# raider99k/UNINA-YOLO-DLA

Hardware: AMD Instinct MI355X
Metric: frames/sec, 640x640 batch-1 (p99 latency alongside) (higher is better)
Workload: dtype f16; 1 GPU; unina-yolo-dla-m graph A fp16, batch=1, 640x640, NMS on-GPU (BASELINE configs[1]); frames_in_flight_per_gpu=2, parallelism=1 GPU, distinct_frames=2048, detections_last_frame=446

## Files before the change

### unina-yolo-dla_amd/csrc/conv_igemm.hip

```cpp
#include "kernels.h"
#include "block_pipeline.h"

#include <cstdlib>

namespace unina {

using namespace dev;

namespace {

typedef float floatx4_t __attribute__((ext_vector_type(4)));

__device__ __forceinline__ void tile_of_block(const ConvParams& p, int orig, int nwg, int* bx, int* by) {
  const int q = nwg >> 3, r = nwg & 7, xcd = orig & 7;
  const int v = (xcd < r ? xcd * (q + 1) : r * (q + 1) + (xcd - r) * q) + (orig >> 3);
  const bool mm = p.xcd_m_major != 0;
  const int major = fast_div(v, mm ? p.gn_magic : p.gm_magic);
  const int minor = v - major * (mm ? p.grid_n : p.grid_m);
  *bx = mm ? major : minor;
  *by = mm ? minor : major;
}

__device__ __forceinline__ void stamp_entry(const ConvParams& p, long long t) {
  if (p.stamps && blockIdx.x == (gridDim.x >> 1) && threadIdx.x == 0) p.stamps[7] = t;
}

__device__ __forceinline__ void stamp_now(const ConvParams& p, int k) {
  p.stamps[k] = __builtin_amdgcn_s_memtime();
  if (k == 0 || k == 4) p.stamps[5 + (k >> 2)] = wall_clock64();
}
__device__ __forceinline__ void stamp(const ConvParams& p, int k) {
  if (p.stamps && blockIdx.x == (gridDim.x >> 1) && threadIdx.x == 0) stamp_now(p, k);
}
__device__ __forceinline__ void stamp(const ConvParams& p, int k, int bid, int nwg) {
  if (p.stamps && bid == (nwg >> 1) && threadIdx.x == 0) stamp_now(p, k);
}

__device__ __forceinline__ void stamp_wg(const ConvParams& p, int which) {
  if (p.wg_times && threadIdx.x == 0) p.wg_times[2 * blockIdx.x + which] = wall_clock64();
}

typedef int intx4 __attribute__((ext_vector_type(4)));
template <typename T> struct Elem;
template <> struct Elem<half_t> {
  static constexpr int kChunk = 8, kBlockK = 32, kPlanes = 1;
  static constexpr int kDType = kF16;
  static constexpr const char* kTag = "f16";
  typedef half8 frag;
  typedef floatx4 acc_t;
  static __device__ __forceinline__ acc_t mma(const frag& a, const frag& b, acc_t c) {
    return __builtin_amdgcn_mfma_f32_16x16x32_f16(a, b, c, 0, 0, 0);
  }
  static __device__ __forceinline__ floatx4 to_float(const acc_t& c) { return c; }
  static __device__ __forceinline__ frag lds(const unsigned char* at, int) { return *reinterpret_cast<const frag*>(at); }
};
template <> struct Elem<s16_t> {
  static constexpr int kChunk = 8, kBlockK = 32, kPlanes = 2;
  static constexpr int kDType = kS16;
  static constexpr const char* kTag = "s16";
  typedef half8x2 frag;
  typedef floatx4 acc_t;
  static __device__ __forceinline__ acc_t mma(const frag& a, const frag& b, acc_t c) { return mfma_split(a, b, c); }
  static __device__ __forceinline__ floatx4 to_float(const acc_t& c) { return c; }
  static __device__ __forceinline__ frag lds(const unsigned char* at, int lo_off) {
    return frag{*reinterpret_cast<const half8*>(at), *reinterpret_cast<const half8*>(at + lo_off)};
  }
};
template <> struct Elem<float> {
  static constexpr int kChunk = 4, kBlockK = 16, kPlanes = 1;
  static constexpr int kDType = kF32;
  static constexpr const char* kTag = "f32";
  static __device__ __forceinline__ floatx4_t lds(const unsigned char* at, int) { return *reinterpret_cast<const floatx4_t*>(at); }
  typedef floatx4_t frag;
  typedef floatx4 acc_t;
  static __device__ __forceinline__ acc_t mma(const frag& a, const frag& b, acc_t c) {
#pragma unroll
    for (int e = 0; e < 4; ++e) c = __builtin_amdgcn_mfma_f32_16x16x4f32(a[e], b[e], c, 0, 0, 0);
    return c;
  }
  static __device__ __forceinline__ floatx4 to_float(const acc_t& c) { return c; }
};
template <> struct Elem<signed char> {
  static constexpr int kChunk = 16, kBlockK = 64, kPlanes = 1;
  static constexpr int kDType = kI8;
// ... 530 lines not shown
      const int h = h00[i] + tap_off;
      hrow[i] = h << (nch_log + 4);
      hsw[i] = h & swz;
    }
#pragma unroll
    for (int j = 0; j < KSUB; ++j) {
      const int ch = (cs * KSUB + j) * 4 + lq;
#pragma unroll
      for (int i = 0; i < WM_T; ++i) f.b[j][i] = *reinterpret_cast<const frag_t*>(patch + hrow[i] + ((ch ^ hsw[i]) << 4));
#pragma unroll
      for (int n = 0; n < WN_T; ++n) f.a[j][n] = *reinterpret_cast<const frag_t*>(sb + (((wn * WN_T + n) * KSUB + j) << 10));
    }
  };
  auto mma_frags = [&](const Frags& f) {
#pragma unroll
    for (int j = 0; j < KSUB; ++j)
#pragma unroll
      for (int n = 0; n < WN_T; ++n)
#pragma unroll
        for (int i = 0; i < WM_T; ++i) acc[n][i] = E::mma(f.a[j][n], f.b[j][i], acc[n][i]);
  };
  EpiConsts<WN_T> ec;
  load_epi_consts<WN_T>(sg, nb0 + wn * (WN_T * 16), lq, ec);
  Frags fa, fb;
  wait_stages<LPT>(n_pro - 1);
  __builtin_amdgcn_s_barrier();
  read_frags(fa, 0);
  stamp(p, 2);
  int kt = 0;
  for (; kt + STAGES < nk; kt += 2) {
    wait_vmcnt<(STAGES - 3) * LPT>();
    __builtin_amdgcn_s_barrier();
    issue((kt + STAGES - 1) % STAGES);
    read_frags(fb, kt + 1);
    mma_frags(fa);
    wait_vmcnt<(STAGES - 3) * LPT>();
    __builtin_amdgcn_s_barrier();
    issue((kt + STAGES) % STAGES);
    read_frags(fa, kt + 2);
    mma_frags(fb);
  }
  bool cur_a = true;
  for (; kt < nk; ++kt) {
    if (kt + 1 < nk) {
      const int issued = kt + STAGES - 1 < nk ? kt + STAGES - 1 : nk;
      wait_stages<LPT>(issued - (kt + 2));
      __builtin_amdgcn_s_barrier();
      if (kt + STAGES - 1 < nk) issue((kt + STAGES - 1) % STAGES);
      if (cur_a) {
        read_frags(fb, kt + 1);
        mma_frags(fa);
      } else {
        read_frags(fa, kt + 1);
        mma_frags(fb);
      }
    } else if (cur_a) {
      mma_frags(fa);
    } else {
      mma_frags(fb);
    }
    cur_a = !cur_a;
  }
  wait_vmcnt<0>();
  stamp(p, 3);

  conv_epilogue<T, BM, BN, WM_T, WN_T>(p, sg, acc, ec, wm, wn, nb0, l15, lq,
                                       [&](int pl) {
                                         const int oy = ty0 + pl / TW, ox = tx0 + pl % TW;
                                         return (oy < p.Ho && ox < p.Wo) ? oy * p.Wo + ox : -1;
                                       },
                                       conv_smem);
  if (p.stamps) {
    asm volatile("s_waitcnt vmcnt(0)" ::: "memory");
    stamp(p, 4);
  }
}
template <typename T, int TH, int TW, int BN, int BK, int WAVES_M, int WAVES_N, int STAGES>
constexpr auto kernel_of(HaloTile<T, TH, TW, BN, BK, WAVES_M, WAVES_N, STAGES>) { return conv3x3_halo<T, TH, TW, BN, BK, WAVES_M, WAVES_N, STAGES>; }

#ifndef UNINA_PATCH_VIA_REGS
#define UNINA_PATCH_VIA_REGS 1
#endif
constexpr bool kPatchViaRegs = UNINA_PATCH_VIA_REGS != 0;
template <typename T, int TH, int TW, int BN, int CIN, int NW, int D, int S = 1>
struct RegqTile : TileDefaults {
  typedef T elem;
  static constexpr int bm = TH * TW, bn = BN, bk = 32, stages = 3, th = TH, tw = TW, cin = CIN, nthreads = NW * 64, stride = S;
  static constexpr int nw = NW, depth = D;
  static constexpr bool SPLIT = Elem<T>::kPlanes == 2;
  static constexpr int R0W = S * (TW - 1) + 3, R0H = S * (TH - 1) + 3;
  static constexpr int PATCH = (int)round_kib(R0H * R0W * CIN * sizeof(T)) + 1024;
  static constexpr int LDS_LO = SPLIT ? PATCH : 0;
  static constexpr size_t lds_bytes(int = 0) { return SPLIT ? 2 * (size_t)PATCH : max_sz(PATCH, stage_bytes((bm + 15) & ~15, BN)); }
  static constexpr Str name() {
    return Str() << "conv3x3_regq<" << Elem<T>::kTag << "," << TH << "x" << TW << "," << BN << "," << CIN << "," << NW << (S == 2 ? "w,s2>" : "w>");
  }
};

template <int TH, int TW, int BN, int CIN, int NW, int D, int S = 1, int WN = 1, typename T = half_t, bool STAMPS = false>
__device__ __forceinline__ void conv3x3_regq_body(const ConvParams& p, int bid, int nwg) {
  typedef Elem<T> E;
  typedef typename E::frag frag;
  typedef RegqTile<T, TH, TW, BN, CIN, NW, D, S> Tile;
  constexpr bool SPLIT = Tile::SPLIT;
  typedef typename std::conditional<sizeof(T) == 1, EltI8, typename std::conditional<SPLIT, EltS, EltH>::type>::type PE;
  constexpr int BM = TH * TW, R0W = Tile::R0W, R0H = Tile::R0H, NT = NW * 64, CB = CIN / E::kBlockK, KB = 9 * CB;
  static_assert(CIN % E::kBlockK == 0, "a weight block must not straddle a tap");
  constexpr int NS = BN / 16 / WN, WVM = NW / NS, MS = (BM + 15) / 16, WM_T = (MS + WVM - 1) / WVM;
  static_assert((BN / 16) % WN == 0 && NW % NS == 0 && WM_T >= 1 && KB * WN >= D, "tile");

  if constexpr (STAMPS) { stamp(p, 0, bid, nwg); stamp_wg(p, 0); }
  const int lane = threadIdx.x & 63;
  const int wid = __builtin_amdgcn_readfirstlane(threadIdx.x >> 6);
  const int wm = wid / NS, wn = wid % NS;
  const int l15 = lane & 15, lq = lane >> 4;
  int bx, by;
  tile_of_block(p, bid, nwg, &bx, &by);
  const int sidx = (p.nseg > 1 && by >= p.seg[1].tile0) ? 1 : 0;
  const ConvSeg& sg = p.seg[sidx];
  const int n_pad = (sg.n_count + 15) & ~15;
  const int nb0 = (by - sg.tile0) * BN;
  const int tiles_x = (p.Wo + TW - 1) / TW;
  const int tyi = fast_div(bx, p.tx_magic), txi = bx - tyi * tiles_x;
  const int ty0 = tyi * TH, tx0 = txi * TW;

  const unsigned char* wptr[WN];
#pragma unroll
  for (int j = 0; j < WN; ++j) {
    int nsub = (nb0 >> 4) + wn * WN + j;
    nsub = nsub * 16 < n_pad ? nsub : (n_pad >> 4) - 1;
    wptr[j] = static_cast<const unsigned char*>(sg.w_lane) + (size_t)nsub * KB * PE::WBLK + lane * 16;
  }
  frag q[D];
  auto fetch = [&](auto gc) {
    constexpr int g = decltype(gc)::value;
    if constexpr (g < KB * WN) q[g % D] = PE::ldw(wptr[g % WN] + (g / WN) * PE::WBLK);
  };
  constexpr int LDS_LO = Tile::LDS_LO;

  constexpr Img X = make_img(0, CIN / E::kChunk);
  if constexpr (SPLIT) {
    load_patch<R0H, R0W, CIN, NT, PE>(conv_smem, static_cast<const T*>(p.src) + sg.src_coff, p.src_ld, p.H, p.W, S * ty0 - 1,
                                      S * tx0 - 1, p.zeros, wid, lane, p.src_lo, LDS_LO);
    static_for<0, D>(fetch);
  } else if constexpr (kPatchViaRegs) {
    PatchRegs<R0H, R0W, CIN, NT, PE> pr;
    patch_issue<R0H, R0W, CIN, NT, PE>(pr, static_cast<const T*>(p.src) + sg.src_coff, p.src_ld, p.H, p.W, S * ty0 - 1, S * tx0 - 1, wid, lane);
    static_for<0, D>(fetch);
    if constexpr (STAMPS) stamp(p, 1, bid, nwg);
    patch_commit<R0H, R0W, CIN, NT, PE>(pr, conv_smem, wid, lane);
  } else {
    load_patch<R0H, R0W, CIN, NT, PE>(conv_smem, static_cast<const T*>(p.src) + sg.src_coff, p.src_ld, p.H, p.W, S * ty0 - 1,
                                      S * tx0 - 1, p.zeros, wid, lane);
    static_for<0, D>(fetch);
  }
  EpiConsts<WN> ec;
  load_epi_consts<WN>(sg, nb0 + wn * (WN * 16), lq, ec);
  if constexpr (STAMPS && (SPLIT || !kPatchViaRegs)) stamp(p, 1, bid, nwg);
  if constexpr (SPLIT || !kPatchViaRegs) asm volatile("s_waitcnt vmcnt(0)" ::: "memory");
  lds_barrier();
  if constexpr (STAMPS) stamp(p, 2, bid, nwg);

  int row0[WM_T];
#pragma unroll
  for (int i = 0; i < WM_T; ++i) {
    int pp = (wm * WM_T + i) * 16 + l15;
    pp = pp < BM ? pp : BM - 1;
    row0[i] = S * ((pp / TW) * R0W + pp % TW);
  }
  auto baddr = [&](int i, auto kc) {
    constexpr int kb = decltype(kc)::value, tap = kb / CB, cb = kb - tap * CB, th3 = tap / 3;
    return X.addr(row0[i] + th3 * R0W + (tap - th3 * 3), cb * 4 + lq);
  };
  typename E::acc_t acc[WN][WM_T];
  frag b[2][WM_T];
#pragma unroll
  for (int i = 0; i < WM_T; ++i) {
#pragma unroll
    for (int j = 0; j < WN; ++j) acc[j][i] = typename E::acc_t{0, 0, 0, 0};
    b[0][i] = PE::ld(conv_smem + baddr(i, std::integral_constant<int, 0>{}), LDS_LO);
  }
  static_for<0, KB>([&](auto kc) {
    constexpr int kb = decltype(kc)::value;
    frag a[WN];
#pragma unroll
    for (int j = 0; j < WN; ++j) a[j] = q[(kb * WN + j) % D];
    static_for<0, WN>([&](auto jc) { fetch(std::integral_constant<int, kb * WN + decltype(jc)::value + D>{}); });
    if constexpr (kb + 1 < KB) {
#pragma unroll
      for (int i = 0; i < WM_T; ++i) b[(kb + 1) & 1][i] = PE::ld(conv_smem + baddr(i, std::integral_constant<int, kb + 1>{}), LDS_LO);
    }
#pragma unroll
    for (int j = 0; j < WN; ++j)
#pragma unroll
      for (int i = 0; i < WM_T; ++i) acc[j][i] = E::mma(a[j], b[kb & 1][i], acc[j][i]);
  });

  if constexpr (STAMPS) stamp(p, 3, bid, nwg);
  auto pix_to_m = [&](int pl) {
    const int oy = ty0 + pl / TW, ox = tx0 + pl % TW;
    return (pl < BM && oy < p.Ho && ox < p.Wo) ? oy * p.Wo + ox : -1;
  };
  conv_epilogue<T, BM, BN, WM_T, WN, decltype(pix_to_m), (UNINA_REGQ_DIRECT_STORE != 0 && sizeof(T) == 2)>(p, sg, acc, ec, wm, wn, nb0, l15, lq, pix_to_m,
                                                                                                       conv_smem, NT);
  if constexpr (STAMPS) { stamp(p, 4, bid, nwg); asm volatile("s_waitcnt vmcnt(0)" ::: "memory"); stamp_wg(p, 1); }
}

template <int TH, int TW, int BN, int CIN, int NW, int D, int S = 1, int WN = 1, typename T = half_t>
__global__ __launch_bounds__(NW * 64) void conv3x3_regq(const ConvParams p) {
  conv3x3_regq_body<TH, TW, BN, CIN, NW, D, S, WN, T>(p, (int)blockIdx.x, (int)gridDim.x);
}
template <typename T, int TH, int TW, int BN, int CIN, int NW, int D, int S>
constexpr auto kernel_of(RegqTile<T, TH, TW, BN, CIN, NW, D, S>) { return conv3x3_regq<TH, TW, BN, CIN, NW, D, S, 1, T>; }

template <typename T, int TH, int CIN, int NCHUNK, int NW>
struct WsTile : TileDefaults {
  typedef T elem;
  static constexpr int TW = 16, BN = NW * 16;
  static constexpr int bm = TH * TW, bn = BN, bk = 32, stages = 3, th = TH, tw = TW, cin = CIN, nthreads = NW * 64, chunks = NCHUNK;
  static constexpr int nw = NW;
  static constexpr bool ws = true;
  static constexpr int ESZ = sizeof(T) == 1 ? 1 : 2;
  static constexpr int R0W = TW + 2, R0H = TH + 2, CC = CIN / NCHUNK;
  static constexpr int PITCH = CC * ESZ + 32;
  static constexpr int PLANE = R0H * R0W * PITCH;
  static constexpr int BUF = Elem<T>::kPlanes * PLANE;
  static constexpr size_t lds_bytes(int = 0) { return (size_t)(NCHUNK > 1 ? 2 : 1) * BUF; }
  static constexpr Str name() {
    return Str() << "conv3x3_ws<" << Elem<T>::kTag << "," << TH << "x16," << CIN << "/" << NCHUNK << "," << NW << "w>";
  }
};

template <typename T, int TH, int CIN, int NCHUNK, int NW, bool STAMPS = false>
__device__ __forceinline__ void conv3x3_wsc_body(const ConvParams& p, int bid, int nwg) {
  typedef Elem<T> E;
  typedef typename E::frag frag;
  typedef WsTile<T, TH, CIN, NCHUNK, NW> Tile;
  constexpr bool SP = E::kPlanes == 2;
  constexpr bool I8 = sizeof(T) == 1;
  constexpr int ESZ = Tile::ESZ, KBLK = E::kBlockK;
  constexpr int WB = 1024 * E::kPlanes;
  if constexpr (STAMPS) { stamp(p, 0, bid, nwg); stamp_wg(p, 0); }
  typedef unsigned uintx4 __attribute__((ext_vector_type(4)));
  typedef float floatx2 __attribute__((ext_vector_type(2)));
  constexpr int TW = Tile::TW, R0W = Tile::R0W, R0H = Tile::R0H, NT = NW * 64, BN = Tile::BN;
  constexpr int CB = CIN / KBLK, CC = Tile::CC, CBC = CC / KBLK, KBC = 9 * CBC;
  constexpr int STEPS = R0H * 3 * CBC, PF = 4;
  constexpr int PITCH = Tile::PITCH, PLANE = Tile::PLANE, BUF = Tile::BUF;
  static_assert(CIN % (KBLK * NCHUNK) == 0 && KBC * 4 * E::kPlanes <= 160 && PLANE % 16 == 0, "chunking: two weight sets must fit the registers");
  static_assert((R0H * R0W + 2) * PITCH < 65536, "ds_read immediate offsets");
  const int lane = threadIdx.x & 63;
  const int wid = __builtin_amdgcn_readfirstlane(threadIdx.x >> 6);
  const int l15 = lane & 15, lq = lane >> 4;
  int bx, by;
  tile_of_block(p, bid, nwg, &bx, &by);
  const int sidx = (p.nseg > 1 && by >= p.seg[1].tile0) ? 1 : 0;
  const ConvSeg& sg = p.seg[sidx];
  const int n_pad = (sg.n_count + 15) & ~15;
  const int nb0 = (by - sg.tile0) * BN;
  const int tiles_x = (p.Wo + TW - 1) / TW;
  const int tyi = fast_div(bx, p.tx_magic), txi = bx - tyi * tiles_x;
  const int ty0 = tyi * TH, tx0 = txi * TW;

  int nsub = (nb0 >> 4) + wid;
  nsub = nsub * 16 < n_pad ? nsub : (n_pad >> 4) - 1;
  const unsigned char* wptr = static_cast<const unsigned char*>(sg.w_lane) + (size_t)nsub * (9 * CB) * WB + lane * 16;
  const int n = nb0 + wid * 16 + lq * 4;
  const bool n_ok = n < sg.n_count;
  const floatx4 bias = *reinterpret_cast<const floatx4*>(sg.bias + (n_ok ? n : 0));

  const int src_bytes = p.H * p.W * p.src_ld * ESZ;
  const __amdgpu_buffer_rsrc_t srs_h = __builtin_amdgcn_make_buffer_rsrc(const_cast<void*>(p.src), 0, src_bytes, 0x00020000);
  const __amdgpu_buffer_rsrc_t srs_l =
      __builtin_amdgcn_make_buffer_rsrc(const_cast<unsigned char*>(static_cast<const unsigned char*>(p.src) + (SP ? p.src_lo : 0)), 0, src_bytes, 0x00020000);
  constexpr int nchx = CC * ESZ / 16, nslots = R0H * R0W * nchx, PITER = (nslots + NT - 1) / NT;

  const bool out16 = !I8 || sg.out_dtype == kF16;
  const int DSZ = out16 ? 2 : 1;
  const unsigned rowb = (unsigned)(p.Wo * sg.dst_ld * DSZ);
  const __amdgpu_buffer_rsrc_t drs_h = __builtin_amdgcn_make_buffer_rsrc(sg.dst, 0, (int)((unsigned)p.Ho * rowb), 0x00020000);
  const __amdgpu_buffer_rsrc_t drs_l =
      __builtin_amdgcn_make_buffer_rsrc(static_cast<unsigned char*>(sg.dst) + (SP ? sg.dst_lo : 0), 0, (int)((unsigned)p.Ho * rowb), 0x00020000);
  const bool lane_ok = n_ok && tx0 + l15 < p.Wo;
  const unsigned voff0 = lane_ok ? (unsigned)(((ty0 * p.Wo + tx0 + l15) * sg.dst_ld + n) * DSZ) : 0x40000000u;
  floatx4 mult = {1.f, 1.f, 1.f, 1.f};
  if constexpr (I8) mult = *reinterpret_cast<const floatx4*>(sg.mult + (n_ok ? n : 0));
  const float out_inv = sg.out_inv_scale;

  typename E::acc_t acc[TH];
  auto store_row = [&](auto rc) {
    constexpr int r = decltype(rc)::value;
    if constexpr (!I8) {
      const floatx4 v = acc[r] + bias;
      half4 hv, lv;
#pragma unroll
      for (int e = 0; e < 4; ++e) {
// ... 101 lines not shown
      }
      if constexpr (s + PF < STEPS) b[(s + PF) % (PF + 1)] = bfrag(std::integral_constant<int, s + PF>{});
      if constexpr (ch == 0 && kx == 0 && cbl == 0 && rho < TH) acc[rho] = typename E::acc_t{0, 0, 0, 0};
      if constexpr (SP) {
        static_for<0, 3>([&](auto tc) {
          constexpr int term = decltype(tc)::value;
          static_for<0, 3>([&](auto kyc) {
            constexpr int ky = decltype(kyc)::value, r = rho - ky;
            if constexpr (r >= 0 && r < TH) {
              const auto& wv = w[(ky * 3 + kx) * CBC + cbl];
              const auto& bv = b[s % (PF + 1)];
              acc[r] = __builtin_amdgcn_mfma_f32_16x16x32_f16(term == 0 ? wv.l : wv.h, term == 1 ? bv.l : bv.h, acc[r], 0, 0, 0);
            }
          });
        });
      } else {
        static_for<0, 3>([&](auto kyc) {
          constexpr int ky = decltype(kyc)::value, r = rho - ky;
          if constexpr (r >= 0 && r < TH) acc[r] = E::mma(w[(ky * 3 + kx) * CBC + cbl], b[s % (PF + 1)], acc[r]);
        });
      }
      if constexpr (ch == NCHUNK - 1 && kx == 1 && cbl == 0 && rho >= 3) store_row(std::integral_constant<int, rho - 3>{});
      __builtin_amdgcn_sched_barrier(0);
    });
    if constexpr (ch + 1 < NCHUNK) {
      patch_commit((ch + 1) & 1);
      lds_barrier();
    }
  });
  if constexpr (STAMPS) stamp(p, 3, bid, nwg);
  store_row(std::integral_constant<int, TH - 1>{});
  if constexpr (STAMPS) { stamp(p, 4, bid, nwg); asm volatile("s_waitcnt vmcnt(0)" ::: "memory"); stamp_wg(p, 1); }
}

template <typename T, int TH, int CIN, int NCHUNK, int NW>
__global__ __launch_bounds__(NW * 64) void conv3x3_wsc(const ConvParams p) {
  conv3x3_wsc_body<T, TH, CIN, NCHUNK, NW>(p, (int)blockIdx.x, (int)gridDim.x);
}
template <typename T, int TH, int CIN, int NCHUNK, int NW>
constexpr auto kernel_of(WsTile<T, TH, CIN, NCHUNK, NW>) { return conv3x3_wsc<T, TH, CIN, NCHUNK, NW>; }

template <typename T> using WsP3 = WsTile<T, 16, 128, (Elem<T>::kPlanes == 2 ? 4 : 2), 4>;
template <typename T> using WsP4 = WsTile<T, 8, 256, 4, 4>;
typedef WsTile<half_t, 8, 128, 2, 4> WsP3Half;
typedef WsTile<half_t, 4, 256, 4, 4> WsP4Half;

template <class A, class B, bool STAMPS = false, int MIN_WAVES = 0>
__global__ __launch_bounds__(A::nthreads, MIN_WAVES) void conv_dual_ws(const ConvParams pa, const ConvParams pb, int nb) {
  if ((int)blockIdx.x < nb) conv3x3_wsc_body<typename B::elem, B::th, B::cin, B::chunks, B::nw, STAMPS>(pb, (int)blockIdx.x, nb);
  else conv3x3_wsc_body<typename A::elem, A::th, A::cin, A::chunks, A::nw, STAMPS>(pa, (int)blockIdx.x - nb, (int)gridDim.x - nb);
}

#ifndef UNINA_CONV_PROBE
template <typename T> using RegqP3 = RegqTile<T, 8, 16, 64, 128, 8, 8>;
template <typename T> using RegqP4 = RegqTile<T, 8, 8, 64, 256, 8, 8>;

template <class A, class B>
__global__ __launch_bounds__(A::nthreads, A::SPLIT ? 0 : 4) void conv_dual_regq(const ConvParams pa, const ConvParams pb, int na) {
  if ((int)blockIdx.x < na) conv3x3_regq_body<A::th, A::tw, A::bn, A::cin, A::nw, A::depth, A::stride, 1, typename A::elem>(pa, (int)blockIdx.x, na);
  else conv3x3_regq_body<B::th, B::tw, B::bn, B::cin, B::nw, B::depth, B::stride, 1, typename B::elem>(pb, (int)blockIdx.x - na, (int)gridDim.x - na);
}

typedef GldsTile<half_t, 128, 16, 64, 4, 1, 4> Head1x1;
__global__ __launch_bounds__(256) void conv_dual_head1x1(const ConvParams pa, const ConvParams pb, int na) {
  if ((int)blockIdx.x < na) conv_glds_body<half_t, 128, 16, 64, 4, 1, 4>(pa, (int)blockIdx.x, na);
  else conv_glds_body<half_t, 128, 16, 64, 4, 1, 4>(pb, (int)blockIdx.x - na, (int)gridDim.x - na);
}

namespace {

constexpr int kCUs = 256;

struct CfgInfo {
  int bm = 0, bn = 0, bk = 0, stages = 0;
  Str name = Str() << "n/a";
  void (*fn)(const ConvParams) = nullptr;
  size_t (*lds_bytes)(int cin) = nullptr;
  int th = 0, tw = 0;
  int cin = 0;
  int nthreads = 0;
  int stride = 0;
  bool ws = false;
  int chunks = 0;
};
struct ConvTable {
  CfgInfo at[kNumDTypes][kCfgCount];
  int clashes = 0;
  template <class Tile>
  constexpr void add(ConvConfig cfg) {
    CfgInfo& c = at[Elem<typename Tile::elem>::kDType][cfg];
    if (c.fn) ++clashes;
    c = {Tile::bm, Tile::bn, Tile::bk, Tile::stages, Tile::name(), kernel_of(Tile{}), &Tile::lds_bytes,
         Tile::th, Tile::tw, Tile::cin, Tile::nthreads, Tile::stride, Tile::ws, Tile::chunks};
  }
};

template <typename T, int ST>
constexpr void add_glds(ConvTable& t) {
  t.add<GldsTile<T, 64, 64, 64, 2, 2, ST>>(kCfg64x64k64);
  t.add<GldsTile<T, 64, 64, 32, 2, 2, 4>>(kCfg64x64k32);
  t.add<GldsTile<T, 128, 64, 64, 2, 2, ST>>(kCfg128x64k64);
  t.add<GldsTile<T, 128, 64, 32, 2, 2, 4>>(kCfg128x64k32);
  t.add<GldsTile<T, 128, 32, 64, 4, 1, ST>>(kCfg128x32k64);
  t.add<GldsTile<T, 128, 32, 32, 4, 1, 4>>(kCfg128x32k32);
  t.add<GldsTile<T, 128, 16, 64, 4, 1, ST>>(kCfg128x16k64);
  t.add<GldsTile<T, 32, 64, 64, 1, 4, 4>>(kCfg32x64k64);
}
template <typename T>
constexpr void add_glds_halo(ConvTable& t) {
  add_glds<T, 4>(t);
  t.add<GldsTile<T, 128, 128, 64, 2, 2, 4>>(kCfg128x128k64);
  t.add<GldsTile<T, 32, 64, 64, 1, 4, 8>>(kCfg32x64k64s8);
  t.add<GldsTile<T, 64, 64, 64, 2, 2, 6>>(kCfg64x64k64s6);
  t.add<HaloTile<T, 8, 8, 64, 64, 2, 2, 4>>(kCfgHalo8x8n64);
  t.add<HaloTile<T, 8, 8, 32, 64, 4, 1, 4>>(kCfgHalo8x8n32);
  t.add<HaloTile<T, 8, 16, 64, 64, 2, 2, 4>>(kCfgHalo8x16n64);
  t.add<HaloTile<T, 8, 16, 32, 64, 4, 1, 4>>(kCfgHalo8x16n32);
  t.add<HaloTile<T, 8, 8, 64, 32, 2, 2, 4>>(kCfgHalo8x8n64k32);
  t.add<HaloTile<T, 8, 16, 32, 32, 4, 1, 4>>(kCfgHalo8x16n32k32);
  t.add<GldsTile<T, 32, 64, 128, 1, 4, 4>>(kCfg32x64k128);
  t.add<GldsTile<T, 64, 64, 128, 2, 2, 4>>(kCfg64x64k128);
}

constexpr ConvTable conv_table() {
  ConvTable t;
  add_glds_halo<half_t>(t);
  add_glds_halo<float>(t);
  add_glds_halo<signed char>(t);
  add_glds<s16_t, 3>(t);

  t.add<RegqTile<half_t, 8, 16, 64, 128, 8, 16>>(kCfgRegq8x16n64c128);
  t.add<RegqTile<half_t, 8, 8, 64, 128, 8, 16>>(kCfgRegq8x8n64c128);
  t.add<RegqTile<half_t, 8, 8, 64, 256, 8, 16>>(kCfgRegq8x8n64c256);
  t.add<RegqTile<half_t, 8, 8, 32, 256, 8, 16>>(kCfgRegq8x8n32c256);
  t.add<RegqTile<half_t, 8, 16, 64, 64, 8, 16>>(kCfgRegq8x16n64c64);
  t.add<RegqTile<half_t, 8, 16, 32, 128, 8, 16>>(kCfgRegq8x16n32c128);
  t.add<RegqTile<half_t, 8, 8, 64, 64, 8, 16, 2>>(kCfgRegqS2_8x8n64c64);
  t.add<RegqTile<half_t, 8, 16, 64, 64, 8, 16, 2>>(kCfgRegqS2_8x16n64c64);
  t.add<RegqTile<half_t, 8, 8, 64, 128, 8, 16, 2>>(kCfgRegqS2_8x8n64c128);
  t.add<RegqTile<half_t, 4, 8, 64, 128, 8, 16, 2>>(kCfgRegqS2_4x8n64c128);
  t.add<RegqTile<half_t, 8, 16, 64, 32, 8, 8, 2>>(kCfgRegqS2_8x16n64c32);
  t.add<RegqTile<half_t, 8, 8, 32, 128, 8, 16, 2>>(kCfgRegqS2_8x8n32c128);
  t.add<RegqTile<signed char, 8, 16, 64, 128, 8, 16>>(kCfgRegq8x16n64c128);
  t.add<RegqTile<signed char, 8, 8, 64, 128, 8, 16>>(kCfgRegq8x8n64c128);
  t.add<RegqTile<signed char, 8, 8, 64, 256, 8, 16>>(kCfgRegq8x8n64c256);
  t.add<RegqTile<signed char, 8, 8, 32, 256, 8, 16>>(kCfgRegq8x8n32c256);
  t.add<RegqTile<signed char, 8, 16, 32, 128, 8, 16>>(kCfgRegq8x16n32c128);
  t.add<RegqTile<signed char, 8, 8, 64, 64, 8, 8, 2>>(kCfgRegqS2_8x8n64c64);
  t.add<RegqTile<signed char, 8, 16, 64, 64, 8, 8, 2>>(kCfgRegqS2_8x16n64c64);
  t.add<RegqTile<signed char, 8, 8, 64, 128, 8, 16, 2>>(kCfgRegqS2_8x8n64c128);
  t.add<RegqTile<signed char, 4, 8, 64, 128, 8, 16, 2>>(kCfgRegqS2_4x8n64c128);
  t.add<RegqTile<signed char, 8, 8, 32, 128, 8, 16, 2>>(kCfgRegqS2_8x8n32c128);
  t.add<RegqTile<s16_t, 8, 16, 64, 128, 8, 8>>(kCfgRegq8x16n64c128);
  t.add<RegqTile<s16_t, 8, 8, 64, 128, 8, 8>>(kCfgRegq8x8n64c128);
  t.add<RegqTile<s16_t, 8, 8, 64, 256, 8, 8>>(kCfgRegq8x8n64c256);
  t.add<RegqTile<s16_t, 8, 16, 64, 64, 8, 8>>(kCfgRegq8x16n64c64);
  t.add<RegqTile<s16_t, 8, 8, 64, 64, 8, 8, 2>>(kCfgRegqS2_8x8n64c64);
  t.add<RegqTile<s16_t, 8, 8, 64, 128, 8, 8, 2>>(kCfgRegqS2_8x8n64c128);
  t.add<RegqTile<s16_t, 4, 8, 64, 128, 8, 8, 2>>(kCfgRegqS2_4x8n64c128);
  t.add<RegqTile<s16_t, 8, 16, 64, 32, 8, 8, 2>>(kCfgRegqS2_8x16n64c32);

  t.add<WsP3<half_t>>(kCfgWs16x16n64c128);
  t.add<WsP4<half_t>>(kCfgWs8x16n64c256);
  t.add<WsP3Half>(kCfgWs8x16n64c128);
  t.add<WsP4Half>(kCfgWs4x16n64c256);
  t.add<WsP3<signed char>>(kCfgWs16x16n64c128);
  t.add<WsP4<signed char>>(kCfgWs8x16n64c256);
  t.add<WsP3<s16_t>>(kCfgWs16x16n64c128);
  t.add<WsTile<s16_t, 16, 64, 2, 4>>(kCfgWsS16x16n64c64);
  t.add<WsTile<s16_t, 8, 128, 2, 4>>(kCfgWsS8x16n64c128);
  t.add<WsP4<s16_t>>(kCfgWsS8x16n64c256);
  return t;
}
constexpr ConvTable kTable = conv_table();
static_assert(kTable.clashes == 0, "two rows of conv_table() name the same (dtype, configuration)");
constexpr const CfgInfo (&kCfg)[kNumDTypes][kCfgCount] = kTable.at;

inline int block_k(int dtype) { return dtype == kF32 ? 16 : (dtype == kI8 ? 64 : 32); }
inline int kstep_of(const ConvParams& p, const CfgInfo& c) { return (c.bk / 32) * block_k(p.dtype); }
inline size_t esize(const ConvParams& p) { return p.dtype == kF32 ? 4 : (p.dtype == kI8 ? 1 : 2); }
inline size_t smem_for(const ConvParams& p, const CfgInfo& c) { return c.lds_bytes(p.Cin); }
int n_tiles(const ConvParams& p, int bn) {
  int t = 0;
  for (int s = 0; s < p.nseg; ++s) t += (((p.seg[s].n_count + 15) & ~15) + bn - 1) / bn;
  return t;
}

dim3 conv_grid(const ConvParams& p, int cfg) {
  const CfgInfo& c = kCfg[p.dtype][cfg];
  if (c.th) return dim3(((p.Ho + c.th - 1) / c.th) * ((p.Wo + c.tw - 1) / c.tw), n_tiles(p, c.bn), 1);
  return dim3((p.M + c.bm - 1) / c.bm, n_tiles(p, c.bn), 1);
}

struct DualKind {
  int cfg_a, cfg_b, threads;
  const char* name;
  void (*fn)(const ConvParams, const ConvParams, int);
  bool b_first;
  int twin;
};
enum { kDualRegq = 0, kDual1x1, kDualRegqI8, kDualWs, kDualWsI8, kDualRegqS16, kDualWsS16, kDualWsSmall, kDualWsStamped, kDualWsS16Stamped,
       kDualKinds };

template <class T>
constexpr int slot_like() {
  for (int i = 0; i < kCfgCount; ++i) {
    const CfgInfo& c = kCfg[Elem<typename T::elem>::kDType][i];
    if (c.fn && c.bm == T::bm && c.bn == T::bn && c.bk == T::bk && c.th == T::th && c.tw == T::tw && c.cin == T::cin && c.nthreads == T::nthreads &&
        c.stride == T::stride && c.ws == T::ws && c.chunks == T::chunks && c.lds_bytes(T::cin) == T::lds_bytes(T::cin))
      return i;
  }
  return -1;
}
template <class A, class B>
constexpr DualKind pair_of(const char* name, void (*fn)(const ConvParams, const ConvParams, int), bool b_first, int twin = -1) {
  static_assert(slot_like<A>() >= 0 && slot_like<B>() >= 0 && A::nthreads == B::nthreads, "a pair's tiles are rows of the table");
  return {slot_like<A>(), slot_like<B>(), A::nthreads, name, fn, b_first, twin};
}
template <typename T> constexpr DualKind regq_pair(const char* name) { return pair_of<RegqP3<T>, RegqP4<T>>(name, conv_dual_regq<RegqP3<T>, RegqP4<T>>, false); }
template <class A, class B, bool STAMPS = false, int MIN_WAVES = 0>
constexpr DualKind ws_pair(const char* name, int twin = -1) { return pair_of<A, B>(name, conv_dual_ws<A, B, STAMPS, MIN_WAVES>, true, twin); }
constexpr DualKind kDual[kDualKinds] = {
    regq_pair<half_t>("conv_dual_head3x3<regq 8x16,64,128 | regq 8x8,64,256>"),
    pair_of<Head1x1, Head1x1>("conv_dual_head1x1<glds 128,16,64 x2>", conv_dual_head1x1, false),
    regq_pair<signed char>("conv_dual_head3x3_i8<regq i8,8x16,64,128 | regq i8,8x8,64,256>"),
    ws_pair<WsP3<half_t>, WsP4<half_t>>("conv_dual_head3x3_ws<ws 16x16,64,128/2 | ws 8x16,64,256/4>", kDualWsStamped),
    ws_pair<WsP3<signed char>, WsP4<signed char>>("conv_dual_head3x3_ws_i8<ws i8,16x16,64,128/2 | ws i8,8x16,64,256/4>"),
    regq_pair<s16_t>("conv_dual_head3x3_s16<regq s16,8x16,64,128 | regq s16,8x8,64,256>"),
    ws_pair<WsP3<s16_t>, WsP4<s16_t>>("conv_dual_head3x3_ws_s16<ws s16,16x16,64,128/4 | ws s16,8x16,64,256/4>", kDualWsS16Stamped),
    ws_pair<WsP3Half, WsP4Half, false, 2>("conv_dual_head3x3_ws_small<ws 8x16,64,128/2 | ws 4x16,64,256/4, 2 per CU>"),
    ws_pair<WsP3<half_t>, WsP4<half_t>, true>("conv_dual_head3x3_ws_stamped<ws 16x16,64,128/2 | ws 8x16,64,256/4>"),
    ws_pair<WsP3<s16_t>, WsP4<s16_t>, true>("conv_dual_head3x3_ws_s16_stamped<ws s16,16x16,64,128/4 | ws s16,8x16,64,256/4>"),
};

}

hipError_t conv_init() {
  for (const auto& row : kCfg) {
    const hipError_t e = set_lds_limits(row);
    if (e != hipSuccess) return e;
  }
  return set_lds_limits(kDual);
}

bool conv_config_valid(const ConvParams& p, int cfg) {
  if (cfg < 0 || cfg >= kCfgCount) return false;
  const CfgInfo& c = kCfg[p.dtype][cfg];
  if (!c.fn) return false;
  if (c.cin) {
    if (p.Cin != c.cin || p.ksize != 3 || p.stride != c.stride || p.pad != 1 || smem_for(p, c) > kMaxLds) return false;
    for (int s = 0; s < p.nseg; ++s)
      if (!p.seg[s].w_lane) return false;
    if (c.ws) {
      if (!p.relu || p.res || !p.zeros) return false;
      for (int s = 0; s < p.nseg; ++s)
        if ((p.seg[s].out_dtype != p.dtype && !(p.dtype == kI8 && p.seg[s].out_dtype == kF16)) || p.seg[s].up2 || p.seg[s].dst_planar ||
            (p.dtype == kI8) != (p.seg[s].mult != nullptr)) return false;
    }
    for (int s = 0; s < p.nseg; ++s)
      if (((p.seg[s].n_count + 15) & ~15) < c.bn) return false;
    return true;
  }
  if (p.Cin % kstep_of(p, c)) return false;
  if (c.th) {
    const int nch = (int)(p.Cin * esize(p) / 16);
    if (p.ksize != 3 || p.stride != 1 || p.pad != 1 || (nch & (nch - 1)) || smem_for(p, c) > kMaxLds) return false;
  }
  int min_npad = 1 << 30;
  for (int s = 0; s < p.nseg; ++s) {
    const int np = (p.seg[s].n_count + 15) & ~15;
    if (np < min_npad) min_npad = np;
  }
  return c.bn <= min_npad || (c.bn == 16);
}

int conv_plan(const ConvParams& p) {
  const int override_cfg = p.force_cfg;
  if (override_cfg >= 0 && conv_config_valid(p, override_cfg)) return override_cfg;
  if (p.dtype == kS16 && p.ksize == 3) {
    for (int c : {(int)kCfgWsS16x16n64c64, (int)kCfgWsS8x16n64c128, (int)kCfgWsS8x16n64c256, (int)kCfgRegqS2_8x16n64c32, (int)kCfgRegqS2_8x8n64c64,
                  (int)kCfgRegqS2_4x8n64c128, (int)kCfgRegq8x16n64c64, (int)kCfgRegq8x16n64c128, (int)kCfgRegq8x8n64c256})
      if (conv_config_valid(p, c)) return c;
  }
  const bool k64 = (p.Cin % (2 * block_k(p.dtype))) == 0;
  int min_npad = 1 << 30;
  for (int s = 0; s < p.nseg; ++s) {
    const int np = (p.seg[s].n_count + 15) & ~15;
    if (np < min_npad) min_npad = np;
  }
  int cfg;
  if (min_npad < 32) cfg = kCfg128x16k64;
  else if (min_npad < 64) cfg = k64 ? kCfg128x32k64 : kCfg128x32k32;
  else {
    auto blocks = [&](int c) { return ((p.M + kCfg[0][c].bm - 1) / kCfg[0][c].bm) * n_tiles(p, kCfg[0][c].bn); };
    const int want = kCUs * 3 / 2;
    if (k64 && min_npad >= 128 && blocks(kCfg128x128k64) >= want) cfg = kCfg128x128k64;
    else if (blocks(k64 ? kCfg128x64k64 : kCfg128x64k32) >= want) cfg = k64 ? kCfg128x64k64 : kCfg128x64k32;
    else if (!k64 || blocks(kCfg64x64k64) >= want || p.M % 64) cfg = k64 ? kCfg64x64k64 : kCfg64x64k32;
    else cfg = kCfg32x64k64;
  }
  if (!conv_config_valid(p, cfg)) cfg = k64 ? kCfg64x64k64 : kCfg64x64k32;
  return cfg;
}

namespace {
int conv_prepare(ConvParams& p, int cfg) {
  const CfgInfo& c = kCfg[p.dtype][cfg];
  const dim3 g = conv_grid(p, cfg);
  p.grid_m = (int)g.x;
  p.gm_magic = div_magic(g.x);
  p.grid_n = (int)g.y;
  p.gn_magic = div_magic(g.y);
  {
    const double in_bytes = (double)esize(p) * p.H * p.W * p.Cin * ((p.nseg > 1 && p.seg[0].src_coff != p.seg[1].src_coff) ? p.nseg : 1);
    double w_bytes = 0;
    for (int s = 0; s < p.nseg; ++s) w_bytes += (double)esize(p) * ((p.seg[s].n_count + 15) & ~15) * p.ksize * p.ksize * p.Cin;
    p.xcd_m_major = (g.x >= 8 && in_bytes + 8.0 * w_bytes < 8.0 * in_bytes + w_bytes) ? 1 : 0;
  }
  p.wo_magic = div_magic((unsigned)p.Wo);
  p.spt_magic = div_magic((unsigned)(p.Cin / kstep_of(p, c)));
  if (c.th) p.tx_magic = div_magic((unsigned)((p.Wo + c.tw - 1) / c.tw));
  int t = 0;
  for (int s = 0; s < p.nseg; ++s) {
    p.seg[s].tile0 = t;
    t += (((p.seg[s].n_count + 15) & ~15) + c.bn - 1) / c.bn;
  }
  return (int)(g.x * g.y);
}
}

hipError_t conv_desc(ConvParams& p, int cfg, LaunchDesc* d) {
  if (cfg < 0 || cfg >= kCfgCount || !kCfg[p.dtype][cfg].fn) return hipErrorInvalidValue;
  const CfgInfo& c = kCfg[p.dtype][cfg];
  const int n = conv_prepare(p, cfg);
  *d = {reinterpret_cast<const void*>(c.fn), dim3(n), dim3(c.nthreads), (unsigned)smem_for(p, c), c.name.s};
  return hipSuccess;
}

int conv_dual_match(const ConvParams& a, const ConvParams& b) {
  if (a.stamps || b.stamps) return -1;
  auto fits = [&](int k) { return a.ksize == 3 && b.ksize == 3 && conv_config_valid(a, kDual[k].cfg_a) && conv_config_valid(b, kDual[k].cfg_b); };
  const char* wsenv = getenv("UNINA_DUAL_WS");
  const bool ws = !(wsenv && wsenv[0] == '0');
  if (a.dtype == kI8 && b.dtype == kI8) {
    if (ws && fits(kDualWsI8)) return kDualWsI8;
    return fits(kDualRegqI8) ? kDualRegqI8 : -1;
  }
  if (a.dtype == kS16 && b.dtype == kS16) {
    if (ws && fits(kDualWsS16)) return kDualWsS16;
    return fits(kDualRegqS16) ? kDualRegqS16 : -1;
  }
  if (a.dtype != kF16 || b.dtype != kF16) return -1;
  if (ws && fits(kDualWs)) {
    const dim3 ga = conv_grid(a, kDual[kDualWs].cfg_a), gb = conv_grid(b, kDual[kDualWs].cfg_b);
    if (fits(kDualWsSmall) && ga.x * ga.y + gb.x * gb.y > kCUs) return kDualWsSmall;
    return kDualWs;
  }
  if (fits(kDualRegq)) return kDualRegq;
  auto tiny = [](const ConvParams& p) {
    for (int s = 0; s < p.nseg; ++s)
      if (p.seg[s].n_count > 16) return false;
    return p.ksize == 1 && p.stride == 1;
  };
  if (tiny(a) && tiny(b) && a.Cin != b.Cin && conv_config_valid(a, kDual[kDual1x1].cfg_a) && conv_config_valid(b, kDual[kDual1x1].cfg_b)) return kDual1x1;
  return -1;
}

hipError_t conv_dual_desc(int kind, ConvParams& a, ConvParams& b, LaunchDesc* d, int* split) {
  if (kind >= 0 && kind < kDualKinds && (a.stamps || b.stamps)) kind = kDual[kind].twin;
  if (kind < 0 || kind >= kDualKinds) return hipErrorInvalidValue;
  const DualKind& k = kDual[kind];
  const int na = conv_prepare(a, k.cfg_a), nb = conv_prepare(b, k.cfg_b);
  *split = k.b_first ? nb : na;
  const size_t smem = max_sz(smem_for(a, kCfg[a.dtype][k.cfg_a]), smem_for(b, kCfg[b.dtype][k.cfg_b]));
  *d = {reinterpret_cast<const void*>(k.fn), dim3(na + nb), dim3(k.threads), (unsigned)smem, k.name};
  return hipSuccess;
}

const char* conv_config_name(int cfg, int dtype) {
  return (cfg >= 0 && cfg < kCfgCount && dtype >= 0 && dtype < kNumDTypes) ? kCfg[dtype][cfg].name.s : "?";
}

}
#else
template __global__ void conv_dual_ws<WsP3<half_t>, WsP4<half_t>>(const ConvParams, const ConvParams, int);
template __global__ void conv_dual_ws<WsP3<signed char>, WsP4<signed char>>(const ConvParams, const ConvParams, int);
template __global__ void conv_dual_ws<WsP3<s16_t>, WsP4<s16_t>>(const ConvParams, const ConvParams, int);
}
#endif
```

Before: 9898 frames/s.

## Add even/odd column-split swizzled LDS patch layout for stride-2 regq convs

For stride-2 3x3 regq convolutions, the input patch is now stored in LDS with even and odd columns split into separate halves, a padded row pitch, and an XOR-like chunk rotation. The goal is to remove LDS bank conflicts when lanes read pixels two columns apart. The epilogue-constant loads are moved to overlap with the patch fetch. A stamped kernel variant is also added for timing probes. The added index arithmetic raises the per-load address cost and makes the layout code more complex.

```diff
diff --git a/unina-yolo-dla_amd/csrc/conv_igemm.hip b/unina-yolo-dla_amd/csrc/conv_igemm.hip
--- a/unina-yolo-dla_amd/csrc/conv_igemm.hip
+++ b/unina-yolo-dla_amd/csrc/conv_igemm.hip
@@ -1,5 +1,6 @@
 #include "kernels.h"
 #include "block_pipeline.h"
+#include "regq_s2.h"
 
 #include <cstdlib>
 
@@ -696,6 +697,9 @@
 #define UNINA_PATCH_VIA_REGS 1
 #endif
 constexpr bool kPatchViaRegs = UNINA_PATCH_VIA_REGS != 0;
+#ifndef UNINA_REGQ_S2_LAYOUT
+#define UNINA_REGQ_S2_LAYOUT 1
+#endif
 template <typename T, int TH, int TW, int BN, int CIN, int NW, int D, int S = 1>
 struct RegqTile : TileDefaults {
   typedef T elem;
@@ -703,20 +707,55 @@
   static constexpr int nw = NW, depth = D;
   static constexpr bool SPLIT = Elem<T>::kPlanes == 2;
   static constexpr int R0W = S * (TW - 1) + 3, R0H = S * (TH - 1) + 3;
-  static constexpr int PATCH = (int)round_kib(R0H * R0W * CIN * sizeof(T)) + 1024;
+  static constexpr bool S2L = S == 2 && !SPLIT && UNINA_REGQ_S2_LAYOUT != 0 && UNINA_PATCH_VIA_REGS != 0;
+  static constexpr int NCH = CIN / Elem<T>::kChunk, S2H = s2::half_w(R0W), S2P = S2L ? s2::pitch(TW, R0W) : R0W;
+  static_assert(!S2L || (s2::nch_ok(NCH) && (TW == 8 || TW == 16)), "regq_s2.h covers 8- and 16-wide tiles of 4, 8 or 16 chunks a pixel");
+  static constexpr int PATCH = (int)round_kib(R0H * S2P * CIN * sizeof(T)) + 1024;
   static constexpr int LDS_LO = SPLIT ? PATCH : 0;
   static constexpr size_t lds_bytes(int = 0) { return SPLIT ? 2 * (size_t)PATCH : max_sz(PATCH, stage_bytes((bm + 15) & ~15, BN)); }
   static constexpr Str name() {
     return Str() << "conv3x3_regq<" << Elem<T>::kTag << "," << TH << "x" << TW << "," << BN << "," << CIN << "," << NW << (S == 2 ? "w,s2>" : "w>");
   }
 };
+
+template <class Tile>
+struct PatchRegsS2 {
+  static constexpr int nreq = s2::requests(Tile::R0H, Tile::R0W, Tile::NCH), ITER = s2::loads(Tile::R0H, Tile::R0W, Tile::NCH, Tile::nthreads);
+  floatx4 v[ITER];
+};
+template <class Tile>
+__device__ __forceinline__ void patch_issue_s2(PatchRegsS2<Tile>& pr, const void* src_, int src_ld, int H, int W, int y0, int x0) {
+  const unsigned char* src = static_cast<const unsigned char*>(src_);
+#pragma unroll
+  for (int it = 0; it < PatchRegsS2<Tile>::ITER; ++it) {
+    const int s = it * Tile::nthreads + (int)threadIdx.x;
+    pr.v[it] = floatx4{0.f, 0.f, 0.f, 0.f};
+    if (s < PatchRegsS2<Tile>::nreq) {
+      const s2::Request r = s2::request(s, Tile::R0W, Tile::NCH);
+      const int iy = y0 + r.ry, ix = x0 + r.rx;
+      if ((unsigned)iy < (unsigned)H && (unsigned)ix < (unsigned)W)
+        pr.v[it] = *reinterpret_cast<const floatx4*>(src + ((size_t)(iy * W + ix) * src_ld) * sizeof(typename Tile::elem) + (r.chunk << 4));
+    }
+  }
+}
+template <class Tile>
+__device__ __forceinline__ void patch_commit_s2(const PatchRegsS2<Tile>& pr, unsigned char* lds_img) {
+#pragma unroll
+  for (int it = 0; it < PatchRegsS2<Tile>::ITER; ++it) {
+    const int s = it * Tile::nthreads + (int)threadIdx.x;
+    if (s < PatchRegsS2<Tile>::nreq) {
+      const s2::Request r = s2::request(s, Tile::R0W, Tile::NCH);
+      *reinterpret_cast<floatx4*>(lds_img + (s2::slot(s2::pixel(r.ry, r.rx, Tile::S2P, Tile::S2H), r.chunk, Tile::NCH) << 4)) = pr.v[it];
+    }
+  }
+}
 
 template <int TH, int TW, int BN, int CIN, int NW, int D, int S = 1, int WN = 1, typename T = half_t, bool STAMPS = false>
 __device__ __forceinline__ void conv3x3_regq_body(const ConvParams& p, int bid, int nwg) {
   typedef Elem<T> E;
   typedef typename E::frag frag;
   typedef RegqTile<T, TH, TW, BN, CIN, NW, D, S> Tile;
-  constexpr bool SPLIT = Tile::SPLIT;
+  constexpr bool SPLIT = Tile::SPLIT, S2L = Tile::S2L;
   typedef typename std::conditional<sizeof(T) == 1, EltI8, typename std::conditional<SPLIT, EltS, EltH>::type>::type PE;
   constexpr int BM = TH * TW, R0W = Tile::R0W, R0H = Tile::R0H, NT = NW * 64, CB = CIN / E::kBlockK, KB = 9 * CB;
   static_assert(CIN % E::kBlockK == 0, "a weight block must not straddle a tap");
@@ -753,7 +792,15 @@
   constexpr int LDS_LO = Tile::LDS_LO;
 
   constexpr Img X = make_img(0, CIN / E::kChunk);
-  if constexpr (SPLIT) {
+  EpiConsts<WN> ec;
+  if constexpr (S2L) {
+    PatchRegsS2<Tile> pr;
+    patch_issue_s2<Tile>(pr, static_cast<const T*>(p.src) + sg.src_coff, p.src_ld, p.H, p.W, S * ty0 - 1, S * tx0 - 1);
+    load_epi_consts<WN>(sg, nb0 + wn * (WN * 16), lq, ec);
+    static_for<0, D>(fetch);
+    if constexpr (STAMPS) stamp(p, 1, bid, nwg);
+    patch_commit_s2<Tile>(pr, conv_smem);
+  } else if constexpr (SPLIT) {
     load_patch<R0H, R0W, CIN, NT, PE>(conv_smem, static_cast<const T*>(p.src) + sg.src_coff, p.src_ld, p.H, p.W, S * ty0 - 1,
                                       S * tx0 - 1, p.zeros, wid, lane, p.src_lo, LDS_LO);
     static_for<0, D>(fetch);
@@ -768,10 +815,9 @@
                                       S * tx0 - 1, p.zeros, wid, lane);
     static_for<0, D>(fetch);
   }
-  EpiConsts<WN> ec;
-  load_epi_consts<WN>(sg, nb0 + wn * (WN * 16), lq, ec);
-  if constexpr (STAMPS && (SPLIT || !kPatchViaRegs)) stamp(p, 1, bid, nwg);
-  if constexpr (SPLIT || !kPatchViaRegs) asm volatile("s_waitcnt vmcnt(0)" ::: "memory");
+  if constexpr (!S2L) load_epi_consts<WN>(sg, nb0 + wn * (WN * 16), lq, ec);
+  if constexpr (STAMPS && !S2L && (SPLIT || !kPatchViaRegs)) stamp(p, 1, bid, nwg);
+  if constexpr (!S2L && (SPLIT || !kPatchViaRegs)) asm volatile("s_waitcnt vmcnt(0)" ::: "memory");
   lds_barrier();
   if constexpr (STAMPS) stamp(p, 2, bid, nwg);
 
@@ -780,11 +826,12 @@
   for (int i = 0; i < WM_T; ++i) {
     int pp = (wm * WM_T + i) * 16 + l15;
     pp = pp < BM ? pp : BM - 1;
-    row0[i] = S * ((pp / TW) * R0W + pp % TW);
+    row0[i] = S2L ? s2::pixel(2 * (pp / TW), 2 * (pp % TW), Tile::S2P, Tile::S2H) : S * ((pp / TW) * R0W + pp % TW);
   }
   auto baddr = [&](int i, auto kc) {
     constexpr int kb = decltype(kc)::value, tap = kb / CB, cb = kb - tap * CB, th3 = tap / 3;
-    return X.addr(row0[i] + th3 * R0W + (tap - th3 * 3), cb * 4 + lq);
+    if constexpr (S2L) return s2::slot(row0[i] + s2::pixel(th3, tap - th3 * 3, Tile::S2P, Tile::S2H), cb * 4 + lq, Tile::NCH) << 4;
+    else return X.addr(row0[i] + th3 * R0W + (tap - th3 * 3), cb * 4 + lq);
   };
   typename E::acc_t acc[WN][WM_T];
   frag b[2][WM_T];
@@ -808,6 +855,7 @@
     for (int j = 0; j < WN; ++j)
 #pragma unroll
       for (int i = 0; i < WM_T; ++i) acc[j][i] = E::mma(a[j], b[kb & 1][i], acc[j][i]);
+    if constexpr (STAMPS && kb == 0) stamp(p, 7, bid, nwg);
   });
 
   if constexpr (STAMPS) stamp(p, 3, bid, nwg);
@@ -817,7 +865,7 @@
   };
   conv_epilogue<T, BM, BN, WM_T, WN, decltype(pix_to_m), (UNINA_REGQ_DIRECT_STORE != 0 && sizeof(T) == 2)>(p, sg, acc, ec, wm, wn, nb0, l15, lq, pix_to_m,
                                                                                                        conv_smem, NT);
-  if constexpr (STAMPS) { stamp(p, 4, bid, nwg); asm volatile("s_waitcnt vmcnt(0)" ::: "memory"); stamp_wg(p, 1); }
+  if constexpr (STAMPS) { asm volatile("s_waitcnt vmcnt(0)" ::: "memory"); stamp(p, 4, bid, nwg); stamp_wg(p, 1); }
 }
 
 template <int TH, int TW, int BN, int CIN, int NW, int D, int S = 1, int WN = 1, typename T = half_t>
@@ -826,6 +874,15 @@
 }
 template <typename T, int TH, int TW, int BN, int CIN, int NW, int D, int S>
 constexpr auto kernel_of(RegqTile<T, TH, TW, BN, CIN, NW, D, S>) { return conv3x3_regq<TH, TW, BN, CIN, NW, D, S, 1, T>; }
+
+template <int TH, int TW, int BN, int CIN, int NW, int D, int S, typename T>
+__global__ __launch_bounds__(NW * 64) void conv3x3_regq_stamped(const ConvParams p) {
+  conv3x3_regq_body<TH, TW, BN, CIN, NW, D, S, 1, T, true>(p, (int)blockIdx.x, (int)gridDim.x);
+}
+template <class Tile>
+constexpr auto stamped_kernel_of(Tile) { return static_cast<void (*)(const ConvParams)>(nullptr); }
+template <int TH, int TW, int BN, int CIN, int NW, int D>
+constexpr auto stamped_kernel_of(RegqTile<half_t, TH, TW, BN, CIN, NW, D, 2>) { return conv3x3_regq_stamped<TH, TW, BN, CIN, NW, D, 2, half_t>; }
 
 template <typename T, int TH, int CIN, int NCHUNK, int NW>
 struct WsTile : TileDefaults {
@@ -1093,6 +1150,7 @@
   int stride = 0;
   bool ws = false;
   int chunks = 0;
+  void (*fn_stamped)(const ConvParams) = nullptr;
 };
 struct ConvTable {
   CfgInfo at[kNumDTypes][kCfgCount];
@@ -1102,7 +1160,7 @@
     CfgInfo& c = at[Elem<typename Tile::elem>::kDType][cfg];
     if (c.fn) ++clashes;
     c = {Tile::bm, Tile::bn, Tile::bk, Tile::stages, Tile::name(), kernel_of(Tile{}), &Tile::lds_bytes,
-         Tile::th, Tile::tw, Tile::cin, Tile::nthreads, Tile::stride, Tile::ws, Tile::chunks};
+         Tile::th, Tile::tw, Tile::cin, Tile::nthreads, Tile::stride, Tile::ws, Tile::chunks, stamped_kernel_of(Tile{})};
   }
 };
 
@@ -1248,7 +1306,9 @@
 
 hipError_t conv_init() {
   for (const auto& row : kCfg) {
-    const hipError_t e = set_lds_limits(row);
+    hipError_t e = set_lds_limits(row);
+    for (const CfgInfo& c : row)
+      if (e == hipSuccess && c.fn_stamped) e = hipFuncSetAttribute(reinterpret_cast<const void*>(c.fn_stamped), hipFuncAttributeMaxDynamicSharedMemorySize, kMaxLds);
     if (e != hipSuccess) return e;
   }
   return set_lds_limits(kDual);
@@ -1344,7 +1404,7 @@
   if (cfg < 0 || cfg >= kCfgCount || !kCfg[p.dtype][cfg].fn) return hipErrorInvalidValue;
   const CfgInfo& c = kCfg[p.dtype][cfg];
   const int n = conv_prepare(p, cfg);
-  *d = {reinterpret_cast<const void*>(c.fn), dim3(n), dim3(c.nthreads), (unsigned)smem_for(p, c), c.name.s};
+  *d = {reinterpret_cast<const void*>(p.stamps && c.fn_stamped ? c.fn_stamped : c.fn), dim3(n), dim3(c.nthreads), (unsigned)smem_for(p, c), c.name.s};
   return hipSuccess;
 }
 
diff --git a/unina-yolo-dla_amd/csrc/regq_s2.h b/unina-yolo-dla_amd/csrc/regq_s2.h
--- /dev/null
+++ b/unina-yolo-dla_amd/csrc/regq_s2.h
@@ -0,0 +1,38 @@
+#pragma once
+
+#if defined(__HIPCC__)
+#define UNINA_S2_HD __host__ __device__
+#else
+#define UNINA_S2_HD
+#endif
+
+namespace unina {
+namespace s2 {
+
+constexpr int half_w(int r0w) { return (r0w + 1) / 2; }
+constexpr int pitch(int tw, int r0w) {
+  int p = 2 * half_w(r0w);
+  if (tw % 16 != 0)
+    while (p % 8 != 4) ++p;
+  return p;
+}
+UNINA_S2_HD constexpr int pixel(int ry, int rx, int pitch_px, int half_px) { return ry * pitch_px + (rx & 1) * half_px + (rx >> 1); }
+UNINA_S2_HD constexpr int slot(int v, int c, int nch) {
+  const int h = nch >> 1, sh = nch == 16 ? 0 : (nch == 8 ? 1 : 2);
+  return v * nch + h * (c & 1) + (((c >> 1) + (v >> sh)) & (h - 1));
+}
+constexpr bool nch_ok(int nch) { return nch == 4 || nch == 8 || nch == 16; }
+constexpr int image_bytes(int r0h, int pitch_px, int nch) { return r0h * pitch_px * nch * 16; }
+
+constexpr int requests(int r0h, int r0w, int nch) { return r0h * r0w * nch; }
+constexpr int loads(int r0h, int r0w, int nch, int nthreads) { return (requests(r0h, r0w, nch) + nthreads - 1) / nthreads; }
+struct Request {
+  int ry, rx, chunk;
+};
+UNINA_S2_HD constexpr Request request(int s, int r0w, int nch) {
+  const int ry = s / (r0w * nch), rem = s - ry * (r0w * nch), rx = rem / nch;
+  return Request{ry, rx, rem - rx * nch};
+}
+
+}
+}
```

Result: faster. 10200 frames/s (median of 6 runs) (+3.1%).
